# PABannier/bark.cpp

Measured on NVIDIA H100. Metric: audio sec/sec (inverse RTF), bark-small f16, batch 1 per GPU, semantic->coarse->fine->encodec, higher is better.
Workload: dtype f16 weights/operands, f32 accumulate (reference arithmetic)

## Files before the change

bark.cpp_b200/csrc/decode_kernels.cu:

```cuda
#include "epilogue.cuh"
#include "gpt_kernels.h"

namespace bark {

namespace {

constexpr int kThreads = 512;
constexpr int kWarps = kThreads / 32;
static_assert(kWarps == 16, "the soft_max tile is 16 columns wide: one warp finishes one column");
constexpr int kWarpSlotBytes = 12 * 1024;
constexpr int kHalfSlotBytes = kWarpSlotBytes / 2;
constexpr int kReplicas = kDecodeReplicas;

struct SmemLayout {
    static constexpr int wslot = 0;
    static constexpr int act = wslot + kWarps * kWarpSlotBytes;
    static constexpr int x = act + 4096 * 4;
    static constexpr int q = x + 1024 * 4;
    static constexpr int part = q + 1024 * 4;
    static constexpr int red = part + (32 * 16 + 128) * 4;
    static constexpr int sched = red + (kWarps + kWarps / 2 + kWarps + 4) * 8;
    static constexpr int total = sched + 128 * 32;
};

__device__ __forceinline__ uint32_t smem_u32(const void * p) { return (uint32_t) __cvta_generic_to_shared(p); }
__device__ __forceinline__ void mbar_init(uint32_t bar, uint32_t count) { asm volatile("mbarrier.init.shared::cta.b64 [%0], %1;" ::"r"(bar), "r"(count)); }
__device__ __forceinline__ void mbar_arrive(uint32_t bar) { asm volatile("mbarrier.arrive.shared::cta.b64 _, [%0];" ::"r"(bar) : "memory"); }
__device__ __forceinline__ void mbar_expect_tx(uint32_t bar, uint32_t bytes) { asm volatile("mbarrier.arrive.expect_tx.shared::cta.b64 _, [%0], %1;" ::"r"(bar), "r"(bytes) : "memory"); }
__device__ __forceinline__ void mbar_wait(uint32_t bar, uint32_t parity) {
    uint32_t done;
    asm volatile("{\n\t.reg .pred p;\n\tmbarrier.try_wait.parity.shared::cta.b64 p, [%1], %2;\n\tselp.u32 %0, 1, 0, p;\n\t}" : "=r"(done) : "r"(bar), "r"(parity) : "memory");
    if (done) return;
    const long long t0 = clock64();
    while (!done) {
        asm volatile("{\n\t.reg .pred p;\n\tmbarrier.try_wait.parity.shared::cta.b64 p, [%1], %2;\n\tselp.u32 %0, 1, 0, p;\n\t}" : "=r"(done) : "r"(bar), "r"(parity) : "memory");
        if (!done && clock64() - t0 > 4000000000ll) __trap();
    }
}
__device__ __forceinline__ void tma_bulk_g2s_stream(uint32_t dst, const void * src, uint32_t bytes, uint32_t bar, unsigned long long policy) {
    asm volatile("cp.async.bulk.shared::cluster.global.mbarrier::complete_tx::bytes.L2::cache_hint [%0], [%1], %2, [%3], %4;"
                 ::"r"(dst), "l"(src), "r"(bytes), "r"(bar), "l"(policy) : "memory");
}
__device__ __forceinline__ unsigned long long l2_evict_first_policy() {
    unsigned long long pol; asm volatile("createpolicy.fractional.L2::evict_first.b64 %0, 1.0;" : "=l"(pol));
    return pol;
}

typedef unsigned long long tagged_t;
__device__ __forceinline__ void publish(tagged_t * p, float v, uint32_t tag) {
    const tagged_t w = ((tagged_t) tag << 32) | (tagged_t) __float_as_uint(v);
    asm volatile("st.relaxed.gpu.global.u64 [%0], %1;" ::"l"(p), "l"(w) : "memory");
}
__device__ __forceinline__ tagged_t peek(const tagged_t * p) {
    tagged_t w;
    asm volatile("ld.relaxed.gpu.global.u64 %0, [%1];" : "=l"(w) : "l"(p) : "memory");
    return w;
}
__device__ __forceinline__ void peek2(const tagged_t * p, tagged_t & a, tagged_t & b) {
    asm volatile("ld.relaxed.gpu.global.v2.u64 {%0, %1}, [%2];" : "=l"(a), "=l"(b) : "l"(p) : "memory");
}
__device__ __forceinline__ void publish_all(tagged_t * base, int n, int i, float v, uint32_t tag, int lane) {
    if (lane < kReplicas) publish(base + (size_t) lane * n + i, v, tag);
}
__shared__ unsigned s_poll_ns;
enum { XT_Q = 0, XT_ATT = 1, XT_X1 = 2, XT_FF = 3, XT_X2 = 4, XT_SC = 5, XT_COUNT = 6 };
__shared__ unsigned s_headstart[XT_COUNT];
__device__ __forceinline__ float consume1(const tagged_t * p, uint32_t tag) {
    tagged_t w = peek(p);
    while ((uint32_t)(w >> 32) != tag) { __nanosleep(s_poll_ns); w = peek(p); }
    return __uint_as_float((uint32_t) w);
}
__device__ __forceinline__ int act_index(int k) {
    const int v = k & 31, c = k >> 5, g = c >> 3, e = c & 7;
    return (((g << 1) + (e >> 2)) * 32 + v) * 4 + (e & 3);
}

__shared__ unsigned long long * s_tim;
__shared__ int s_tim_layer, s_tim_tid;
template <bool TM>
__device__ __forceinline__ void tstamp(int i) {
    if (TM && s_tim && (int) threadIdx.x == s_tim_tid) {
        unsigned long long t; asm volatile("mov.u64 %0, %%globaltimer;" : "=l"(t));
        const int layer = s_tim_layer;
        if (blockIdx.x == 0) s_tim[layer * 32 + i] = t;
        if (layer == 5) s_tim[(64 + blockIdx.x) * 32 + i] = t;
    }
}

template <bool TM>
__device__ __forceinline__ void tstamp2(int row0, int i) {
    if (TM && s_tim && (int) threadIdx.x == s_tim_tid && blockIdx.x == 0 && s_tim_layer < 16) {
        unsigned long long t; asm volatile("mov.u64 %0, %%globaltimer;" : "=l"(t));
        s_tim[(row0 + s_tim_layer) * 32 + i] = t;
    }
}

enum { SINK_PLAIN = 0, SINK_ACT = 1, SINK_ACT_R16 = 2 };
template <int MAXJ>
__device__ __forceinline__ void consume_to_smem_inl(const tagged_t * g, int n, uint32_t tag, float * dst, int mode, int xt) {
    constexpr int PJ = MAXJ / 2;
    tagged_t w[PJ][2];
    g += (size_t)(blockIdx.x % kReplicas) * n;
    const unsigned hs = s_headstart[xt];
    if (hs) __nanosleep(hs);
#pragma unroll
    for (int j = 0; j < PJ; j++) { const int i = 2 * (threadIdx.x + j * kThreads); if (i < n) peek2(g + i, w[j][0], w[j][1]); }
#pragma unroll
    for (int j = 0; j < PJ; j++) {
        const int i = 2 * (threadIdx.x + j * kThreads);
        if (i < n) {
            while ((uint32_t)(w[j][0] >> 32) != tag || (uint32_t)(w[j][1] >> 32) != tag) { __nanosleep(s_poll_ns); peek2(g + i, w[j][0], w[j][1]); }
#pragma unroll
            for (int e = 0; e < 2; e++) {
                const float v = __uint_as_float((uint32_t) w[j][e]);
                if (mode == SINK_PLAIN) dst[i + e] = v; else dst[act_index(i + e)] = mode == SINK_ACT_R16 ? round_f16(v) : v;
            }
        }
    }
    __syncthreads();
}
__device__ __forceinline__ void consume_row_to_smem(const tagged_t * g, int n, uint32_t tag, float * dst) {
    tagged_t w[2];
    const unsigned hs = s_headstart[XT_SC];
    if (hs) __nanosleep(hs);
#pragma unroll
    for (int j = 0; j < 2; j++) { const int i = threadIdx.x + j * kThreads; if (i < n) w[j] = peek(g + i); }
#pragma unroll
    for (int j = 0; j < 2; j++) {
        const int i = threadIdx.x + j * kThreads;
        if (i < n) {
            while ((uint32_t)(w[j] >> 32) != tag) { __nanosleep(s_poll_ns); w[j] = peek(g + i); }
            dst[i] = __uint_as_float((uint32_t) w[j]);
        }
    }
    __syncthreads();
}
template <int MAXJ>
__device__ __noinline__ void consume_to_smem(const tagged_t * g, int n, uint32_t tag, float * dst, int mode, int xt) {
    consume_to_smem_inl<MAXJ>(g, n, tag, dst, mode, xt);
}


__device__ __forceinline__ double approx_rcp(double x) {
    double y = (double) __frcp_rn((float) x);
    double e = __fma_rn(-x, y, 1.0); y = __fma_rn(y, e, y);
    e = __fma_rn(-x, y, 1.0);        y = __fma_rn(y, e, y);
    return y;
}

template <bool ROUND16, bool TM, bool NATURAL = false, int COPY = 0>
__device__ __noinline__ void block_layernorm(const float * xs, int E, double inv_E, const float * __restrict__ g, const float * __restrict__ b, float * act,
                                             double * red, unsigned * fallback_counter, int sb) {
    const int tid = threadIdx.x, lane = tid & 31, warp = tid >> 5;
    const int tb = sb == 1 ? 0 : 16;
    tstamp2<TM>(48, tb + 0);
    double * sA = red, * sB = red + kWarps + kWarps / 2;
    float * fA = reinterpret_cast<float *>(red + kWarps);
    const int i0 = tid, i1 = tid + kThreads;
    const bool h0 = i0 < E, h1 = i1 < E;
    const float g0 = h0 ? __ldg(g + i0) : 0.f, g1 = h1 ? __ldg(g + i1) : 0.f;
    const float b0 = (b && h0) ? __ldg(b + i0) : 0.f, b1 = (b && h1) ? __ldg(b + i1) : 0.f;
    const float x0 = h0 ? xs[i0] : 0.f, x1 = h1 ? xs[i1] : 0.f;
    const double slack = 2.0 * (double) E * 0x1p-53 * (1.0 + 1e-6);

    double s = (double) x0 + (double) x1;
    float a = fabsf(x0) + fabsf(x1);
#pragma unroll
    for (int o = 16; o > 0; o >>= 1) { s += __shfl_xor_sync(0xffffffffu, s, o); a += __shfl_xor_sync(0xffffffffu, a, o); }
    tstamp2<TM>(48, tb + 1);
    if (lane == 0) { sA[warp] = s; fA[warp] = a; }
    __syncthreads();
    tstamp2<TM>(48, tb + 2);
    float mean;
    {
        double qd[1]; float qf[1];
        qd[0] = sA[lane & (kWarps - 1)]; qf[0] = fA[lane & (kWarps - 1)];
#pragma unroll
        for (int o = kWarps / 2; o > 0; o >>= 1) { qd[0] += __shfl_xor_sync(0xffffffffu, qd[0], o); qf[0] += __shfl_xor_sync(0xffffffffu, qf[0], o); }
        const double S = qd[0]; const float A = qf[0];
        if (S == 1.25) tstamp2<TM>(48, tb + 15);
        tstamp2<TM>(48, tb + 3);
        const double c = S * inv_E;
        const double hw = (slack * (double) A * 1.001) * inv_E + fabs(c) * 0x1p-50;
        mean = __double2float_rn(c - hw);
        if (mean != __double2float_rn(c + hw)) {
            double ss = 0.0;
            for (int i = 0; i < E; i++) ss = __dadd_rn(ss, (double) xs[i]);
            mean = __double2float_rn(__ddiv_rn(ss, (double) E));
            if (fallback_counter && tid == 0) atomicAdd(fallback_counter, 1u);
        }
    }
    tstamp<TM>(sb);
    const float v0 = __fsub_rn(x0, mean), v1 = __fsub_rn(x1, mean);
    double s2 = (h0 ? (double) __fmul_rn(v0, v0) : 0.0) + (h1 ? (double) __fmul_rn(v1, v1) : 0.0);
#pragma unroll
    for (int o = 16; o > 0; o >>= 1) s2 += __shfl_xor_sync(0xffffffffu, s2, o);
    if (s2 == 1.25) tstamp2<TM>(48, tb + 15);
    tstamp2<TM>(48, tb + 5);
    if (lane == 0) sB[warp] = s2;
    __syncthreads();
    tstamp2<TM>(48, tb + 6);
    float scale;
    {
        double qd[1];
        qd[0] = sB[lane & (kWarps - 1)];
#pragma unroll
        for (int o = kWarps / 2; o > 0; o >>= 1) qd[0] += __shfl_xor_sync(0xffffffffu, qd[0], o);
        const double S2 = qd[0];
        const double c = S2 * inv_E;
        const double hw = (slack * S2) * inv_E + c * 0x1p-50;
        float variance = __double2float_rn(c - hw);
        if (variance != __double2float_rn(c + hw)) {
            double ss = 0.0;
            for (int i = 0; i < E; i++) { const float v = __fsub_rn(xs[i], mean); ss = __dadd_rn(ss, (double) __fmul_rn(v, v)); }
            variance = __double2float_rn(__ddiv_rn(ss, (double) E));
            if (fallback_counter && tid == 0) atomicAdd(fallback_counter, 1u);
        }
        scale = __fdiv_rn(1.0f, __fsqrt_rn(__fadd_rn(variance, 1e-5f)));
    }
    if (scale == 1.25f) tstamp2<TM>(48, tb + 15);
    tstamp2<TM>(48, tb + 7);
    if (h0) { float y = __fmul_rn(__fmul_rn(v0, scale), g0); if (b) y = __fadd_rn(y, b0); act[NATURAL ? i0 : act_index(i0)] = ROUND16 ? round_f16(y) : y; }
    if (h1) { float y = __fmul_rn(__fmul_rn(v1, scale), g1); if (b) y = __fadd_rn(y, b1); act[NATURAL ? i1 : act_index(i1)] = ROUND16 ? round_f16(y) : y; }
    tstamp2<TM>(48, tb + 8);
    __syncthreads();
    tstamp2<TM>(48, tb + 9);
}

struct PhaseSched { int r0, r1, K, row_bytes; const unsigned char * w; const unsigned char * ws; };

enum { EP_QKV = 0, EP_RESID = 1, EP_GELU = 2, EP_LOGITS = 3 };

__device__ __forceinline__ float gelu_sel(float v, __half t) { return v <= -10.0f ? 0.0f : v >= 10.0f ? v : __half2float(t); }

template <typename WT> struct Unpack;
template <> struct Unpack<__half> {
    static constexpr int G = 8;
    __device__ static void w(const uint4 & u, float (&f)[8]) {
        const __half2 * h = reinterpret_cast<const __half2 *>(&u);
#pragma unroll
        for (int i = 0; i < 4; i++) { const float2 t = __half22float2(h[i]); f[2 * i] = t.x; f[2 * i + 1] = t.y; }
    }
};
template <> struct Unpack<float> {
    static constexpr int G = 4;
    __device__ static void w(const uint4 & u, float (&f)[4]) { f[0] = __uint_as_float(u.x); f[1] = __uint_as_float(u.y); f[2] = __uint_as_float(u.z); f[3] = __uint_as_float(u.w); }
};

__device__ __forceinline__ uint4 lds128(uint32_t addr) {
    uint4 v; asm volatile("ld.shared.v4.u32 {%0, %1, %2, %3}, [%4];" : "=r"(v.x), "=r"(v.y), "=r"(v.z), "=r"(v.w) : "r"(addr));
    return v;
}
template <typename WT, bool SH, int NR>
__device__ __forceinline__ void row_dot(const unsigned char * row, int row_bytes, const float * act, int K, int lane, float (&out)[NR]) {
    constexpr int G = Unpack<WT>::G;
    const int nsteps = K >> 5;
    const uint4 * wv = reinterpret_cast<const uint4 *>(row) + lane;
    const uint32_t sw = SH ? smem_u32(row) + lane * 16 : 0u;
    const int rstride = row_bytes >> 4;
    auto fetch = [&](int n, int i) -> uint4 { return SH ? lds128(sw + n * row_bytes + i * 512) : wv[n * rstride + i * 32]; };
    float acc[NR];
#pragma unroll
    for (int n = 0; n < NR; n++) acc[n] = 0.0f;
    if constexpr (G == 8) {
        const int ng = nsteps >> 3, tail = nsteps & 7;
#pragma unroll 3
        for (int g = 0; g < ng; g++) {
            const float4 a0 = *reinterpret_cast<const float4 *>(act + ((g * 2) * 32 + lane) * 4);
            const float4 a1 = *reinterpret_cast<const float4 *>(act + ((g * 2 + 1) * 32 + lane) * 4);
#pragma unroll
            for (int n = 0; n < NR; n++) {
                float w[8]; Unpack<WT>::w(fetch(n, g), w);
                float c = acc[n];
                c = __fmaf_rn(w[0], a0.x, c); c = __fmaf_rn(w[1], a0.y, c); c = __fmaf_rn(w[2], a0.z, c); c = __fmaf_rn(w[3], a0.w, c);
                c = __fmaf_rn(w[4], a1.x, c); c = __fmaf_rn(w[5], a1.y, c); c = __fmaf_rn(w[6], a1.z, c); c = __fmaf_rn(w[7], a1.w, c);
                acc[n] = c;
            }
        }
        if (tail) {
            const float * a0 = act + ((ng * 2) * 32 + lane) * 4, * a1 = act + ((ng * 2 + 1) * 32 + lane) * 4;
#pragma unroll
            for (int n = 0; n < NR; n++) {
                float w[8]; Unpack<WT>::w(fetch(n, ng), w);
#pragma unroll
                for (int e = 0; e < 8; e++) if (e < tail) acc[n] = __fmaf_rn(w[e], e < 4 ? a0[e] : a1[e - 4], acc[n]);
            }
        }
    } else {
        const int nq = nsteps >> 2, tail = nsteps & 3;
        for (int qd = 0; qd < nq; qd++) {
            const float4 a = *reinterpret_cast<const float4 *>(act + (qd * 32 + lane) * 4);
#pragma unroll
            for (int n = 0; n < NR; n++) {
                float w[4]; Unpack<WT>::w(fetch(n, qd), w);
                float c = acc[n];
                c = __fmaf_rn(w[0], a.x, c); c = __fmaf_rn(w[1], a.y, c); c = __fmaf_rn(w[2], a.z, c); c = __fmaf_rn(w[3], a.w, c);
                acc[n] = c;
            }
        }
        if (tail) {
            const float * a = act + (nq * 32 + lane) * 4;
#pragma unroll
            for (int n = 0; n < NR; n++) {
                float w[4]; Unpack<WT>::w(fetch(n, nq), w);
#pragma unroll
                for (int e = 0; e < 4; e++) if (e < tail) acc[n] = __fmaf_rn(w[e], a[e], acc[n]);
            }
        }
    }
#pragma unroll
    for (int n = 0; n < NR; n++) out[n] = lane_tree_reduce(acc[n]);
}

struct Q4 {};
template <typename WT> struct IsQ4 { static constexpr bool v = false; };
template <> struct IsQ4<Q4> { static constexpr bool v = true; };

__device__ __forceinline__ void quantize_act_q8(const float * act, int K, int8_t * q, float * d) {
    const int lane = threadIdx.x & 31, warp = threadIdx.x >> 5;
    for (int b = warp; b < (K >> 5); b += kWarps) {
        const float v = act[b * 32 + lane];
        float amax = fabsf(v);
#pragma unroll
        for (int o = 16; o > 0; o >>= 1) amax = fmaxf(amax, __shfl_xor_sync(0xffffffffu, amax, o));
        const float id = amax != 0.0f ? __fdiv_rn(127.0f, amax) : 0.0f;
        const float p = __fmul_rn(v, id);
        q[b * 32 + lane] = (int8_t)(isfinite(p) ? __float2int_rn(p) : -128);
        if (lane == 0) d[b] = __half2float(__float2half_rn(__fdiv_rn(amax, 127.0f)));
    }
    __syncthreads();
}

template <bool SH>
__device__ __forceinline__ float row_dot_q4(const unsigned char * qrows, const unsigned char * srows, int nrows, int nb, const int8_t * aq, const float * ad, int lane) {
    const int l = lane & 7, row = min(lane >> 3, nrows - 1);
    const bool high = l >= 4;
    const unsigned char * wq = qrows + (size_t) row * nb * 16 + (l & 3) * 4;
    const unsigned char * ws = srows + (size_t) row * nb * 2;
    const uint32_t s_wq = SH ? smem_u32(wq) : 0u, s_ws = SH ? smem_u32(ws) : 0u, s_aq = smem_u32(aq) + l * 4, s_ad = smem_u32(ad);
    float acc = 0.0f;
    constexpr int UB = 8;
    for (int b0 = 0; b0 < nb; b0 += UB) {
        uint32_t wr[UB]; float dr[UB]; int yr[UB];
#pragma unroll
        for (int u = 0; u < UB; u++) if (b0 + u < nb) {
            unsigned short hs; float da;
            if (SH) { asm volatile("ld.shared.u32 %0, [%1];" : "=r"(wr[u]) : "r"(s_wq + (b0 + u) * 16) : "memory"); asm volatile("ld.shared.u16 %0, [%1];" : "=h"(hs) : "r"(s_ws + (b0 + u) * 2) : "memory"); }
            else    { wr[u] = __ldg(reinterpret_cast<const uint32_t *>(wq + (size_t)(b0 + u) * 16)); hs = __ldg(reinterpret_cast<const unsigned short *>(ws + (size_t)(b0 + u) * 2)); }
            asm volatile("ld.shared.f32 %0, [%1];" : "=f"(da) : "r"(s_ad + (b0 + u) * 4) : "memory");
            asm volatile("ld.shared.s32 %0, [%1];" : "=r"(yr[u]) : "r"(s_aq + (b0 + u) * 32) : "memory");
            dr[u] = __fmul_rn(__half2float(__ushort_as_half(hs)), da);
        }
#pragma unroll
        for (int u = 0; u < UB; u++) {
            if (b0 + u < nb) {
                const uint32_t w = (high ? (wr[u] >> 4) : wr[u]) & 0x0f0f0f0fu;
                const int wi = (int) __vsub4(w, 0x08080808u);
                acc = __fmaf_rn(dr[u], (float) __dp4a(wi, yr[u], 0), acc);
            }
        }
    }
    acc = __fadd_rn(acc, __shfl_xor_sync(0xffffffffu, acc, 4));
    acc = __fadd_rn(acc, __shfl_xor_sync(0xffffffffu, acc, 2));
    acc = __fadd_rn(acc, __shfl_xor_sync(0xffffffffu, acc, 1));
    return acc;
}
__device__ __forceinline__ float wte_q4_value(const void * wte, int E, int row, int i) {
    const unsigned char * blk = (const unsigned char *) wte + ((size_t) row * (E >> 5) + (i >> 5)) * 18;
    const float d = __half2float(__ushort_as_half((unsigned short)(blk[0] | (blk[1] << 8))));
    const int j = i & 31, q = j < 16 ? (blk[2 + j] & 0x0f) : (blk[2 + j - 16] >> 4);
    return __fmul_rn((float)(q - 8), d);
}

template <typename WT>
__device__ __forceinline__ void embed_token(const void * wte, const float * wpe, const int32_t * token_ptr, int token, int n_vocab_in, int E, int n_past, float * xs) {
    if (token_ptr) token = min(max(__ldcg(token_ptr), 0), n_vocab_in - 1);
    for (int i = threadIdx.x; i < E; i += kThreads) {
        float t;
        if constexpr (IsQ4<WT>::v) t = wte_q4_value(wte, E, token, i);
        else t = (float) ((const WT *) wte)[(size_t) token * E + i];
        xs[i] = __fadd_rn(t, wpe[(size_t) n_past * E + i]);
    }
}

constexpr int kMaxTasks = 8;

struct BlockCtx {
    tagged_t * gq, * gk, * gv, * gx, * gff, * gatt, * gscores;
    float * mem_k, * mem_v, * logits;
    const __half * gelu_tab;
    unsigned long long policy;
    int E, ctx, n_past, n_phases;
    float scale;
};
__shared__ BlockCtx s_bc;
__shared__ __align__(8) unsigned long long s_bar[kWarps][2];
extern __shared__ __align__(128) unsigned char dsm[];

__device__ __forceinline__ const PhaseSched * sched_tab() { return reinterpret_cast<const PhaseSched *>(dsm + SmemLayout::sched); }
__device__ __forceinline__ void warp_rows(const PhaseSched & p, int warp, int & a, int & b) {
    const int n = p.r1 - p.r0;
    a = p.r0 + ((warp * n) >> 4); b = p.r0 + (((warp + 1) * n) >> 4);
}

__device__ __forceinline__ bool q4_staged(uint32_t qbytes, uint32_t sbytes, const unsigned char * ssrc) {
    return qbytes != 0 && qbytes + sbytes <= (uint32_t) kHalfSlotBytes && (sbytes & 15u) == 0 && (reinterpret_cast<uintptr_t>(ssrc) & 15u) == 0;
}

__device__ __forceinline__ void stage_rows(int phase) {
    if (phase >= s_bc.n_phases || (threadIdx.x & 31) != 0) return;
    const int warp = threadIdx.x >> 5, half = phase & 1;
    const PhaseSched p = sched_tab()[phase];
    int a, b; warp_rows(p, warp, a, b);
    const uint32_t bytes = (uint32_t)((b - a) * p.row_bytes);
    const uint32_t bar = smem_u32(&s_bar[warp][half]);
    const uint32_t dst = smem_u32(dsm + SmemLayout::wslot) + warp * kWarpSlotBytes + half * kHalfSlotBytes;
    if (p.ws) {
        const uint32_t sbytes = (uint32_t)((b - a) * (p.K >> 5) * 2);
        const unsigned char * ssrc = p.ws + (size_t) a * (p.K >> 5) * 2;
        if (q4_staged(bytes, sbytes, ssrc)) {
            asm volatile("fence.proxy.async.shared::cta;" ::: "memory");
            mbar_expect_tx(bar, bytes + sbytes);
            tma_bulk_g2s_stream(dst, p.w + (size_t) a * p.row_bytes, bytes, bar, s_bc.policy);
            tma_bulk_g2s_stream(dst + bytes, ssrc, sbytes, bar, s_bc.policy);
        } else {
            mbar_arrive(bar);
        }
        return;
    }
    if (bytes != 0 && bytes <= (uint32_t) kHalfSlotBytes) {
        asm volatile("fence.proxy.async.shared::cta;" ::: "memory");
        mbar_expect_tx(bar, bytes);
        tma_bulk_g2s_stream(dst, p.w + (size_t) a * p.row_bytes, bytes, bar, s_bc.policy);
    } else {
        mbar_arrive(bar);
    }
}

__device__ __forceinline__ uint32_t staged_bytes_of(int phase, int warp) {
    const PhaseSched p = sched_tab()[phase];
    int a, b; warp_rows(p, warp, a, b);
    const uint32_t bytes = (uint32_t)((b - a) * p.row_bytes);
    if (p.ws) {
        const uint32_t sbytes = (uint32_t)((b - a) * (p.K >> 5) * 2);
        return q4_staged(bytes, sbytes, p.ws + (size_t) a * (p.K >> 5) * 2) ? bytes + sbytes : 0u;
    }
    return bytes <= (uint32_t) kHalfSlotBytes ? bytes : 0u;
}
__device__ __forceinline__ void cp_async_16(uint32_t dst, const float * src) { asm volatile("cp.async.cg.shared.global [%0], [%1], 16;" ::"r"(dst), "l"(src) : "memory"); }
__device__ __forceinline__ void cp_async_commit() { asm volatile("cp.async.commit_group;" ::: "memory"); }
__device__ __forceinline__ void cp_async_wait_all() { asm volatile("cp.async.wait_group 0;" ::: "memory"); }

template <typename WT, bool TM>
__device__ __noinline__ void run_phase(int phase, int ep, int layer, uint32_t otag, int sb) {
    const int lane = threadIdx.x & 31, warp = threadIdx.x >> 5;
    const int tb = sb == 3 ? 0 : sb == 18 ? 8 : sb == 24 ? 16 : 24;
    tstamp2<TM>(32, tb + 0);
    const PhaseSched p = sched_tab()[phase];
    const float * act = reinterpret_cast<const float *>(dsm + SmemLayout::act);
    const float * xs = reinterpret_cast<const float *>(dsm + SmemLayout::x);
    const int half = phase & 1;
    int a, b; warp_rows(p, warp, a, b);
    const uint32_t bytes = (uint32_t)((b - a) * p.row_bytes);
    const bool staged = bytes != 0 && bytes <= (uint32_t) kHalfSlotBytes;
    const unsigned char * slot = dsm + SmemLayout::wslot + (size_t) warp * kWarpSlotBytes + (size_t) half * kHalfSlotBytes;
    mbar_wait(smem_u32(&s_bar[warp][half]), (uint32_t)(phase >> 1) & 1u);
    tstamp<TM>(sb);
    const int E = s_bc.E;
    auto emit = [&](int r, float v) {
        if (ep == EP_QKV) {
            const size_t slot_off = ((size_t) layer * s_bc.ctx + s_bc.n_past) * E;
            if (r < E) publish_all(s_bc.gq, E, r, v, otag, lane);
            else if (lane == 0) {
                if (r < 2 * E) { publish(s_bc.gk + (r - E), v, otag); s_bc.mem_k[slot_off + (r - E)] = v; }
                else           { publish(s_bc.gv + (r - 2 * E), v, otag); s_bc.mem_v[slot_off + (r - 2 * E)] = v; }
            }
        } else if (ep == EP_RESID) {
            publish_all(s_bc.gx, E, r, __fadd_rn(v, xs[r]), otag, lane);
        } else if (lane == 0) {
            s_bc.logits[r] = v;
        }
    };
    if constexpr (IsQ4<WT>::v) {
        const int nb = p.K >> 5;
        const int8_t * aq = reinterpret_cast<const int8_t *>(dsm + SmemLayout::q);
        const float * ad = reinterpret_cast<const float *>(dsm + SmemLayout::part) + 512;
        const uint32_t sbytes = (uint32_t)((b - a) * nb * 2);
        const unsigned char * ssrc = p.ws + (size_t) a * nb * 2;
        const bool st4 = q4_staged(bytes, sbytes, ssrc);
        for (int r = a; r < b; r += 4) {
            const int n = min(4, b - r);
            const float t = st4 ? row_dot_q4<true>(slot + (size_t)(r - a) * p.row_bytes, slot + bytes + (size_t)(r - a) * nb * 2, n, nb, aq, ad, lane)
                                : row_dot_q4<false>(p.w + (size_t) r * p.row_bytes, p.ws + (size_t) r * nb * 2, n, nb, aq, ad, lane);
#pragma unroll
            for (int g = 0; g < 4; g++) {
                const float v = __shfl_sync(0xffffffffu, t, g * 8);
                if (g < n && lane < kReplicas) {
                    if (ep == EP_GELU) publish_all(s_bc.gff, 4 * E, r + g, gelu_sel(v, s_bc.gelu_tab[__half_as_ushort(__float2half_rn(v))]), otag, lane);
                    else emit(r + g, v);
                }
            }
        }
        __syncwarp();
        tstamp<TM>(sb + 1);
        return;
    } else {
    int j = 0;
    tstamp2<TM>(32, tb + 1);
    for (int r = a; r < b;) {
        const unsigned char * row = staged ? slot + (size_t) j * p.row_bytes : p.w + (size_t) r * p.row_bytes;
        if (r + 1 < b) {
            float v[2];
            if (staged) row_dot<WT, true, 2>(row, p.row_bytes, act, p.K, lane, v);
            else { float u[1]; row_dot<WT, false, 1>(row, p.row_bytes, act, p.K, lane, u); v[0] = u[0]; row_dot<WT, false, 1>(row + p.row_bytes, p.row_bytes, act, p.K, lane, u); v[1] = u[0]; }
            if (v[0] == 1.2345e30f) tstamp2<TM>(32, tb + 7);
            tstamp2<TM>(32, tb + 2);
            if (lane < kReplicas) {
                if (ep == EP_GELU) {
                    const __half t0 = s_bc.gelu_tab[__half_as_ushort(__float2half_rn(v[0]))], t1 = s_bc.gelu_tab[__half_as_ushort(__float2half_rn(v[1]))];
                    publish_all(s_bc.gff, 4 * E, r, gelu_sel(v[0], t0), otag, lane); publish_all(s_bc.gff, 4 * E, r + 1, gelu_sel(v[1], t1), otag, lane);
                } else { emit(r, v[0]); emit(r + 1, v[1]); }
            }
            tstamp2<TM>(32, tb + 3);
            r += 2; j += 2;
        } else {
            float v[1];
            if (staged) row_dot<WT, true, 1>(row, p.row_bytes, act, p.K, lane, v); else row_dot<WT, false, 1>(row, p.row_bytes, act, p.K, lane, v);
            if (v[0] == 1.2345e30f) tstamp2<TM>(32, tb + 7);
            tstamp2<TM>(32, tb + 4);
            if (lane < kReplicas) {
                if (ep == EP_GELU) publish_all(s_bc.gff, 4 * E, r, gelu_sel(v[0], s_bc.gelu_tab[__half_as_ushort(__float2half_rn(v[0]))]), otag, lane);
                else emit(r, v[0]);
            }
            tstamp2<TM>(32, tb + 5);
            r += 1; j += 1;
        }
    }
    __syncwarp();
    tstamp<TM>(sb + 1);
    }
}

}

template <int DSTEPS>
__device__ __forceinline__ void key_tail(int warp, uint32_t & off, int & cap) {
    constexpr int D = DSTEPS * 32;
    off = (max(staged_bytes_of(0, warp), staged_bytes_of(2, warp)) + 127u) & ~127u;
    cap = min(2 * kMaxTasks, (int)(((uint32_t) kHalfSlotBytes - min(off, (uint32_t) kHalfSlotBytes)) / (uint32_t)(D * 4)));
}

template <int DSTEPS>
__device__ __noinline__ void p2_stage_keys(int layer, int H, int n_kv, unsigned score_cta0) {
    constexpr int D = DSTEPS * 32, GPT = D / 4;
    const int lane = threadIdx.x & 31, warp = threadIdx.x >> 5;
    const int E = s_bc.E, ctx = s_bc.ctx, n_past = s_bc.n_past;
    uint32_t off; int cap; key_tail<DSTEPS>(warp, off, cap);
    const float * Kc = s_bc.mem_k + (size_t) layer * ctx * E;
    const int total = H * n_past, gw = (int)(blockIdx.x - score_cta0) * kWarps + warp, nw = (int)(gridDim.x - score_cta0) * kWarps;
    const uint32_t dst = smem_u32(dsm + SmemLayout::wslot + (size_t) warp * kWarpSlotBytes + off);
#pragma unroll 2
    for (int q = lane; q < cap * GPT; q += 32) {
        const int i = q / GPT, g = q - i * GPT, t = gw + i * nw;
        if (t < total) {
            const int h = t / n_past, k = t - h * n_past;
            cp_async_16(dst + (uint32_t) q * 16u, Kc + (size_t) k * E + h * D + g * 4);
        }
    }
    cp_async_commit();
}

template <int DSTEPS, bool TM>
__device__ __noinline__ void p2_scores(int il, int H, int n_kv, uint32_t t_qkv, uint32_t t_sc, unsigned score_cta0) {
    constexpr int D = DSTEPS * 32;
    const int lane = threadIdx.x & 31, warp = threadIdx.x >> 5;
    const int E = s_bc.E, ctx = s_bc.ctx, n_past = s_bc.n_past;
    const float scale = s_bc.scale;
    float * qs = reinterpret_cast<float *>(dsm + SmemLayout::q);
    const float * Kc = s_bc.mem_k + (size_t) il * ctx * E;
    const int total = H * n_past, gw = (int)(blockIdx.x - score_cta0) * kWarps + warp, nw = (int)(gridDim.x - score_cta0) * kWarps;
    const int sq = nw / n_past, sr = nw - sq * n_past;
    uint32_t off; int cap; key_tail<DSTEPS>(warp, off, cap);
    if (score_cta0 == 0) cap = 0;
    const float * ks = reinterpret_cast<const float *>(dsm + SmemLayout::wslot + (size_t) warp * kWarpSlotBytes + off) + lane;
    tstamp<TM>(6);
    consume_to_smem<2>(s_bc.gq, E, t_qkv, qs, SINK_PLAIN, XT_Q);
    tstamp<TM>(7);
    if (cap > 0) { cp_async_wait_all(); __syncwarp(); }
    int h = gw / n_past, k = gw - h * n_past;
    int done = 0;
#pragma unroll 1
    for (int b0 = 0; b0 < cap && gw + b0 * nw < total; b0 += kMaxTasks) {
        float r[kMaxTasks];
#pragma unroll
        for (int i = 0; i < kMaxTasks; i++) {
            float acc = 0.0f;
            if (b0 + i < cap && h < H) {
#pragma unroll
                for (int c = 0; c < DSTEPS; c++) acc = __fmaf_rn(ks[(b0 + i) * D + c * 32], qs[h * D + c * 32 + lane], acc);
            }
            r[i] = acc;
            k += sr; h += sq; if (k >= n_past) { k -= n_past; h++; }
        }
        static_assert(kMaxTasks == 8, "the transposed butterfly below is written for eight tasks");
        const bool u16 = (lane & 16) != 0, u8 = (lane & 8) != 0, u4 = (lane & 4) != 0;
#pragma unroll
        for (int i = 0; i < 4; i++) { const float keep = u16 ? r[i + 4] : r[i], send = u16 ? r[i] : r[i + 4]; r[i] = __fadd_rn(keep, __shfl_xor_sync(0xffffffffu, send, 16)); }
#pragma unroll
        for (int i = 0; i < 2; i++) { const float keep = u8 ? r[i + 2] : r[i], send = u8 ? r[i] : r[i + 2]; r[i] = __fadd_rn(keep, __shfl_xor_sync(0xffffffffu, send, 8)); }
        { const float keep = u4 ? r[1] : r[0], send = u4 ? r[0] : r[1]; r[0] = __fadd_rn(keep, __shfl_xor_sync(0xffffffffu, send, 4)); }
        r[0] = __fadd_rn(r[0], __shfl_xor_sync(0xffffffffu, r[0], 1));
        r[0] = __fadd_rn(r[0], __shfl_xor_sync(0xffffffffu, r[0], 2));
        const int mine = b0 + (u16 ? 4 : 0) + (u8 ? 2 : 0) + (u4 ? 1 : 0);
        const int t = gw + mine * nw;
        if ((lane & 3) == 0 && mine < cap && t < total) {
            const int hh = t / n_past, kk = t - hh * n_past;
            publish(s_bc.gscores + (size_t) hh * ctx + kk, __fmul_rn(r[0], scale), t_sc);
        }
        done = min(b0 + kMaxTasks, cap);
    }
#pragma unroll 1
    for (int t = gw + done * nw; t < total; t += nw) {
        const int hh = t / n_past, kk = t - hh * n_past;
        float acc = 0.0f;
#pragma unroll
        for (int c = 0; c < DSTEPS; c++) acc = __fmaf_rn(__ldcg(Kc + (size_t) kk * E + hh * D + c * 32 + lane), qs[hh * D + c * 32 + lane], acc);
        const float rr = lane_tree_reduce(acc);
        if (lane == 0) publish(s_bc.gscores + (size_t) hh * ctx + kk, __fmul_rn(rr, scale), t_sc);
    }
#pragma unroll 1
    for (int hh = gw; hh < H; hh += nw) {
        float acc = 0.0f;
#pragma unroll
        for (int c = 0; c < DSTEPS; c++) acc = __fmaf_rn(consume1(s_bc.gk + hh * D + c * 32 + lane, t_qkv), qs[hh * D + c * 32 + lane], acc);
        const float rr = lane_tree_reduce(acc);
        if (lane == 0) publish(s_bc.gscores + (size_t) hh * ctx + n_past, __fmul_rn(rr, scale), t_sc);
    }
}

template <bool TM>
__device__ __forceinline__ float softmax_exp_rcp(float * p, int n_kv, double * red, unsigned * fallbacks) {
    const int tid = threadIdx.x, lane = tid & 31, warp = tid >> 5;
    float * bc = reinterpret_cast<float *>(red + kWarps + kWarps / 2 + kWarps);
    float mx = __int_as_float(0xff800000);
#pragma unroll 1
    for (int i = tid; i < n_kv; i += kThreads) mx = fmaxf(mx, p[i]);
#pragma unroll
    for (int o = 16; o > 0; o >>= 1) mx = fmaxf(mx, __shfl_xor_sync(0xffffffffu, mx, o));
    float * fred = reinterpret_cast<float *>(red);
    if (lane == 0) fred[warp] = mx;
    __syncthreads();
    mx = fred[0];
#pragma unroll
    for (int w = 1; w < kWarps; w++) mx = fmaxf(mx, fred[w]);
    tstamp<TM>(11);
    const int nchunks = n_kv >> 3, n8 = nchunks << 3;
#pragma unroll 1
    for (int i = tid; i < n_kv; i += kThreads) {
        const float d = __fsub_rn(p[i], mx);
        p[i] = i < n8 ? ggml_v_expf_dev(d) : glibc_expf_dev(d);
    }
    __syncthreads();
    tstamp<TM>(12);
    if (warp == 0) {
        auto chunk_sum = [&](int c) {
            const float4 lo4 = *reinterpret_cast<const float4 *>(p + c * 8), hi4 = *reinterpret_cast<const float4 *>(p + c * 8 + 4);
            const float t0 = __fadd_rn(hi4.x, lo4.x), t1 = __fadd_rn(hi4.y, lo4.y), t2 = __fadd_rn(hi4.z, lo4.z), t3 = __fadd_rn(hi4.w, lo4.w);
            return __fadd_rn(__fadd_rn(t0, t2), __fadd_rn(t1, t3));
        };
        double s = 0.0;
#pragma unroll 1
        for (int c = lane; c < nchunks; c += 32) s += (double) chunk_sum(c);
#pragma unroll
        for (int o = 16; o > 0; o >>= 1) s += __shfl_xor_sync(0xffffffffu, s, o);
        if (lane == 0) {
            const double dl = 2.0 * (double)(nchunks + 8) * 0x1p-53 * s * (1.0 + 1e-6);
            double lo = s - dl, hi = s + dl;
#pragma unroll 1
            for (int i = n8; i < n_kv; i++) { const double tl = (double) p[i]; lo = __dadd_rn(lo, tl); hi = __dadd_rn(hi, tl); }
            const double mid = 0.5 * (lo + hi), y = approx_rcp(mid);
            const double rw = (hi - lo) * y * 0.5 + 0x1p-48;
            float f_lo = __double2float_rn(y * (1.0 - rw));
            const float f_hi = __double2float_rn(y * (1.0 + rw));
            if (f_lo != f_hi) {
                double q2 = 0.0;
#pragma unroll 1
                for (int c = 0; c < nchunks; c++) q2 = __dadd_rn(q2, (double) chunk_sum(c));
#pragma unroll 1
                for (int i = n8; i < n_kv; i++) q2 = __dadd_rn(q2, (double) p[i]);
                f_lo = __double2float_rn(__ddiv_rn(1.0, q2));
                if (fallbacks) atomicAdd(fallbacks + 1, 1u);
            }
            bc[2] = f_lo;
        }
    }
    __syncthreads();
    tstamp<TM>(13);
    return bc[2];
}

template <int DSTEPS, bool TM>
__device__ __noinline__ void p3_attention(int il, int n_kv, uint32_t t_qkv, uint32_t t_sc, uint32_t t_att, unsigned * ln_fallbacks) {
    constexpr int D = DSTEPS * 32;
    const int tid = threadIdx.x, lane = tid & 31, warp = tid >> 5;
    const int E = s_bc.E, ctx = s_bc.ctx, n_past = s_bc.n_past;
    float * act = reinterpret_cast<float *>(dsm + SmemLayout::act);
    float * qs = reinterpret_cast<float *>(dsm + SmemLayout::q);
    float * part = reinterpret_cast<float *>(dsm + SmemLayout::part);
    double * red = reinterpret_cast<double *>(dsm + SmemLayout::red);
    struct { float * mem_v; unsigned * ln_fallbacks; } A{s_bc.mem_v, ln_fallbacks};
    constexpr int parts = D >> 4;
    const int pv_h = blockIdx.x / parts, pv_c = blockIdx.x % parts, np = n_kv & ~31;
    const int v = tid >> 4, dd = tid & 15, h = pv_h;
    const int col0 = pv_h * D + pv_c * 16;
    const int nstep = np >> 5, r = n_kv - np;
    const int nstep_all = nstep + (r > 0 ? 1 : 0);
    const float * Vt = A.mem_v + (size_t) il * ctx * E + col0;
    const uint32_t voff = (staged_bytes_of(4 * il + 1, warp) + 127u) & ~127u;
    const bool vs_ok = voff + (uint32_t) nstep_all * 128u <= (uint32_t) kHalfSlotBytes;
    const float * vs = reinterpret_cast<const float *>(dsm + SmemLayout::wslot + (size_t) warp * kWarpSlotBytes + kHalfSlotBytes + voff);
    if (vs_ok) {
        const uint32_t dst = smem_u32(vs);
        const int sub = lane >> 3, vl2 = (lane >> 2) & 1, g = lane & 3;
#pragma unroll 2
        for (int c0 = 0; c0 < nstep_all; c0 += 4) {
            const int c = c0 + sub, k = 2 * warp + vl2 + 32 * c;
            if (c < nstep_all && k < n_past) cp_async_16(dst + (uint32_t)(((c * 2 + vl2) * 16 + g * 4) * 4), Vt + (size_t) k * E + g * 4);
        }
        cp_async_commit();
    }
    const float v_new = consume1(s_bc.gv + col0 + dd, t_qkv);
    __syncthreads();
    tstamp<TM>(9);
    float * p = qs;
    consume_row_to_smem(s_bc.gscores + (size_t) h * ctx, n_kv, t_sc, p);
    tstamp<TM>(10);
    const float sc_f = softmax_exp_rcp<TM>(p, n_kv, red, A.ln_fallbacks);
    float acc = 0.0f;
    if (vs_ok) {
        cp_async_wait_all(); __syncwarp();
#pragma unroll 8
        for (int c = 0; c < nstep; c++) {
            const int k = v + 32 * c;
            const float vv = k < n_past ? vs[c * 32 + lane] : v_new;
            acc = __fmaf_rn(vv, __fmul_rn(p[k], sc_f), acc);
        }
    } else {
#pragma unroll 8
        for (int c = 0; c < nstep; c++) {
            const int k = v + 32 * c;
            const float vv = k < n_past ? __ldcg(Vt + (size_t) k * E + dd) : v_new;
            acc = __fmaf_rn(vv, __fmul_rn(p[k], sc_f), acc);
        }
    }
    part[v * 17 + dd] = acc;
    const int r8 = r & ~7, n4 = r8 + ((r - r8) >= 4 ? 4 : 0);
    if (v < r) {
        const float vv = (np + v < n_past) ? (vs_ok ? vs[nstep * 32 + lane] : __ldcg(Vt + (size_t)(np + v) * E + dd)) : v_new;
        act[v * 16 + dd] = v < n4 ? __fmul_rn(vv, __fmul_rn(p[np + v], sc_f)) : vv;
    }
    __syncthreads();
    tstamp<TM>(15);
    {
        float sum = lane_tree_reduce(part[lane * 17 + warp]);
#pragma unroll 8
        for (int j = 0; j < n4; j++) sum = __fadd_rn(sum, act[j * 16 + warp]);
#pragma unroll 1
        for (int j = n4; j < r; j++) sum = __fmaf_rn(act[j * 16 + warp], __fmul_rn(p[np + j], sc_f), sum);
        publish_all(s_bc.gatt, E, col0 + warp, sum, t_att, lane);
    }
    __syncthreads();
}

template <typename WT, int DSTEPS, bool TM>
__global__ void __launch_bounds__(kThreads, 1) gpt_decode_step_kernel(DecodeArgs A) {
    float * act = reinterpret_cast<float *>(dsm + SmemLayout::act);
    float * xs = reinterpret_cast<float *>(dsm + SmemLayout::x);
    float * qs = reinterpret_cast<float *>(dsm + SmemLayout::q);
    float * part = reinterpret_cast<float *>(dsm + SmemLayout::part);
    double * red = reinterpret_cast<double *>(dsm + SmemLayout::red);
    float * bc = reinterpret_cast<float *>(red + kWarps + kWarps / 2 + kWarps);
    const int tid = threadIdx.x, lane = tid & 31, warp = tid >> 5;
    constexpr int D = DSTEPS * 32;
    const int E = A.E, H = A.H, L = A.L, ctx = A.block_size, n_past = A.n_past, n_kv = n_past + 1;
    constexpr bool kQ4 = IsQ4<WT>::v;
    constexpr bool kRound = !kQ4 && sizeof(WT) == 2;
    constexpr int kSinkAct = kQ4 ? SINK_PLAIN : kRound ? SINK_ACT_R16 : SINK_ACT;
    int8_t * act_q = reinterpret_cast<int8_t *>(dsm + SmemLayout::q);
    float * act_d = reinterpret_cast<float *>(dsm + SmemLayout::part) + 512;

    PhaseSched * sched = reinterpret_cast<PhaseSched *>(dsm + SmemLayout::sched);
    const int n_phases = 4 * L + 1;
    if (tid < n_phases) {
        const DecodePhase ph = A.phases[tid];
        int lo = 0, hi = ph.n_out;
        if (tid == n_phases - 1) { lo = A.lm_lo; hi = A.lm_hi; }
        const int n = hi - lo, G = gridDim.x, base = n / G, rem = n % G, cta = blockIdx.x;
        PhaseSched e;
        e.r0 = lo + cta * base + min(cta, rem); e.r1 = e.r0 + base + (cta < rem ? 1 : 0);
        e.K = ph.K; e.row_bytes = ph.row_bytes; e.w = (const unsigned char *) ph.w; e.ws = (const unsigned char *) ph.ws;
        sched[tid] = e;
    }
    if (tid == kThreads - 1) {
        s_bc.gq = (tagged_t *) A.gq; s_bc.gk = (tagged_t *) A.gk; s_bc.gv = (tagged_t *) A.gv; s_bc.gx = (tagged_t *) A.gx; s_bc.gff = (tagged_t *) A.gff;
        s_bc.gatt = (tagged_t *) A.gatt; s_bc.gscores = (tagged_t *) A.gscores;
        s_bc.mem_k = A.mem_k; s_bc.mem_v = A.mem_v; s_bc.logits = A.logits; s_bc.gelu_tab = A.gelu_tab;
        s_bc.policy = l2_evict_first_policy();
        s_bc.E = E; s_bc.ctx = ctx; s_bc.n_past = n_past; s_bc.n_phases = n_phases; s_bc.scale = 1.0f / sqrtf((float) E / (float) H);
        s_tim = A.timing; s_tim_layer = 0; s_tim_tid = A.timing_tid; s_poll_ns = A.poll_ns;
    }
    if (tid < XT_COUNT) {
        const bool pv = (int) blockIdx.x < A.H * ((A.E / A.H) >> 4);
        s_headstart[tid] = (tid == XT_ATT && pv) ? 0u : A.headstart[tid];
    }
    if (lane == 0) {
        mbar_init(smem_u32(&s_bar[warp][0]), 1); mbar_init(smem_u32(&s_bar[warp][1]), 1);
        asm volatile("fence.mbarrier_init.release.cluster;" ::: "memory");
    }
    __syncthreads();
    stage_rows(0);
    stage_rows(1);

    embed_token<WT>(A.wte, A.wpe, A.token_ptr, A.token, A.n_vocab_in, E, n_past, xs);
    __syncthreads();

    uint32_t tag = A.tag_base;
    const double inv_E = A.inv_E;

    const int parts = D >> 4;
    const bool pv_cta = (int) blockIdx.x < H * parts;
    const unsigned score_cta0 = (gridDim.x >= (unsigned)(H * parts + 64)) ? (unsigned)(H * parts) : 0u;
    const bool score_cta = blockIdx.x >= score_cta0;

    if (score_cta0 != 0 && score_cta) p2_stage_keys<DSTEPS>(0, H, n_kv, score_cta0);
#pragma unroll 1
    for (int il = 0; il < L; il++) {
        const DecodeLayerVec lv = A.layer_vecs[il];
        const uint32_t t_qkv = tag + 1, t_sc = tag + 2, t_att = tag + 3, t_x1 = tag + 4, t_ff = tag + 5, t_x2 = tag + 6;
        tag += 6;
        if (tid == A.timing_tid) s_tim_layer = il;
        tstamp<TM>(0);
        block_layernorm<kRound, TM, kQ4>(xs, E, inv_E, lv.ln_1_g, lv.ln_1_b, act, red, A.ln_fallbacks, 1);
        if constexpr (kQ4) quantize_act_q8(act, E, act_q, act_d);
        tstamp<TM>(2);
        run_phase<WT, TM>(4 * il + 0, EP_QKV, il, t_qkv, 3);

        if constexpr (kQ4) __syncthreads();
        if (score_cta) {
            p2_scores<DSTEPS, TM>(il, H, n_kv, t_qkv, t_sc, score_cta0);
            tstamp<TM>(8);
            if (score_cta0 != 0 && il + 1 < L) p2_stage_keys<DSTEPS>(il + 1, H, n_kv, score_cta0);
        } else {
            tstamp<TM>(8);
        }
        if (pv_cta) p3_attention<DSTEPS, TM>(il, n_kv, t_qkv, t_sc, t_att, A.ln_fallbacks);
        tstamp<TM>(16);
        stage_rows(4 * il + 2);

        consume_to_smem<2>(s_bc.gatt, E, t_att, act, kSinkAct, XT_ATT);
        if constexpr (kQ4) quantize_act_q8(act, E, act_q, act_d);
        tstamp<TM>(17);
        run_phase<WT, TM>(4 * il + 1, EP_RESID, il, t_x1, 18);

        consume_to_smem<2>(s_bc.gx, E, t_x1, xs, SINK_PLAIN, XT_X1);
        stage_rows(4 * il + 3);
        tstamp<TM>(21);
        block_layernorm<kRound, TM, kQ4>(xs, E, inv_E, lv.ln_2_g, lv.ln_2_b, act, red, A.ln_fallbacks, 22);
        if constexpr (kQ4) quantize_act_q8(act, E, act_q, act_d);
        tstamp<TM>(23);
        run_phase<WT, TM>(4 * il + 2, EP_GELU, il, t_ff, 24);
        __syncthreads();
        tstamp<TM>(27);

        consume_to_smem<8>(s_bc.gff, 4 * E, t_ff, act, kSinkAct, XT_FF);
        stage_rows(4 * il + 4);
        if constexpr (kQ4) quantize_act_q8(act, 4 * E, act_q, act_d);
        tstamp<TM>(28);
        run_phase<WT, TM>(4 * il + 3, EP_RESID, il, t_x2, 29);

        consume_to_smem<2>(s_bc.gx, E, t_x2, xs, SINK_PLAIN, XT_X2);
        stage_rows(4 * il + 5);
        tstamp<TM>(14);
    }
    if (tid == A.timing_tid) s_tim_layer = L;
    tstamp<TM>(0);
    block_layernorm<kRound, TM, kQ4>(xs, E, inv_E, A.ln_f_g, A.ln_f_b, act, red, A.ln_fallbacks, 1);
    if constexpr (kQ4) quantize_act_q8(act, E, act_q, act_d);
    tstamp<TM>(2);
    run_phase<WT, TM>(4 * L, EP_LOGITS, 0, 0, 3);
}

__global__ void __launch_bounds__(kThreads) decode_rows_kernel(int op, const float * __restrict__ x, int n, double inv_n, const float * __restrict__ g,
                                                               const float * __restrict__ b, float * __restrict__ out, unsigned * counters) {
    __shared__ double red[kWarps + kWarps / 2 + kWarps + 4];
    __shared__ __align__(16) float p[1024];
    const float * xr = x + (size_t) blockIdx.x * n;
    float * orow = out + (size_t) blockIdx.x * n;
    if (op == 0) { block_layernorm<false, false, true, 1>(xr, n, inv_n, g, b, orow, red, counters, 1); return; }
    for (int i = threadIdx.x; i < n; i += kThreads) p[i] = xr[i];
    __syncthreads();
    const float sc_f = softmax_exp_rcp<false>(p, n, red, counters);
    for (int i = threadIdx.x; i < n; i += kThreads) orow[i] = __fmul_rn(p[i], sc_f);
}

void decode_rows(int op, const float * x, int rows, int n, const float * g, const float * b, float * out, unsigned * counters, cudaStream_t s) {
    BARK_LAUNCH(decode_rows_kernel, rows, kThreads, 0, s, op, x, n, 1.0 / n, g, b, out, counters);
}

template <bool SH>
__global__ void __launch_bounds__(kThreads) decode_q4_rows_kernel(const float * __restrict__ x, int K, const unsigned char * __restrict__ wq,
                                                                  const unsigned char * __restrict__ ws, int n_out, MatmulEpilogue ep,
                                                                  int8_t * __restrict__ q_out, float * __restrict__ d_out) {
    const int lane = threadIdx.x & 31, warp = threadIdx.x >> 5, nb = K >> 5;
    int8_t * aq = reinterpret_cast<int8_t *>(dsm);
    float * ad = reinterpret_cast<float *>(dsm + K);
    unsigned char * slot = dsm + K + nb * 4 + (size_t) warp * 4 * nb * 18;
    quantize_act_q8(x, K, aq, ad);
    for (int i = threadIdx.x; i < K; i += kThreads) q_out[i] = aq[i];
    for (int i = threadIdx.x; i < nb; i += kThreads) d_out[i] = ad[i];
    for (int r = warp * 4; r < n_out; r += kWarps * 4) {
        const int n = min(4, n_out - r);
        float t;
        if constexpr (SH) {
            const uint32_t * src = reinterpret_cast<const uint32_t *>(wq + (size_t) r * nb * 16);
            const unsigned short * ssrc = reinterpret_cast<const unsigned short *>(ws + (size_t) r * nb * 2);
            for (int i = lane; i < n * nb * 4; i += 32) reinterpret_cast<uint32_t *>(slot)[i] = src[i];
            for (int i = lane; i < n * nb; i += 32) reinterpret_cast<unsigned short *>(slot + n * nb * 16)[i] = ssrc[i];
            __syncwarp();
            t = row_dot_q4<true>(slot, slot + n * nb * 16, n, nb, aq, ad, lane);
            __syncwarp();
        } else {
            t = row_dot_q4<false>(wq + (size_t) r * nb * 16, ws + (size_t) r * nb * 2, n, nb, aq, ad, lane);
        }
#pragma unroll
        for (int g = 0; g < 4; g++) {
            const float v = __shfl_sync(0xffffffffu, t, g * 8);
            if (lane == 0 && g < n) matmul_epilogue(ep, 0, r + g, v);
        }
    }
}

void decode_q4_rows(bool staged, const float * x, int K, const void * qs, const void * scales, int n_out, const MatmulEpilogue & ep, int8_t * q_out,
                    float * d_out, cudaStream_t s) {
    const size_t smem = (size_t) K + (K >> 5) * 4 + (staged ? (size_t) kWarps * 4 * (K >> 5) * 18 : 0);
    const unsigned char * wq = (const unsigned char *) qs, * ws = (const unsigned char *) scales;
    if (staged) {
        BARK_CUDA_CHECK(cudaFuncSetAttribute(decode_q4_rows_kernel<true>, cudaFuncAttributeMaxDynamicSharedMemorySize, (int) smem));
        BARK_LAUNCH(decode_q4_rows_kernel<true>, 1, kThreads, smem, s, x, K, wq, ws, n_out, ep, q_out, d_out);
    } else {
        BARK_LAUNCH(decode_q4_rows_kernel<false>, 1, kThreads, smem, s, x, K, wq, ws, n_out, ep, q_out, d_out);
    }
}

static size_t decode_smem_bytes() { return (size_t) SmemLayout::total + 128; }

int decode_tags_per_step(int n_layer) { return 6 * n_layer; }

template <typename WT, int DSTEPS, bool TM>
static void launch_variant(DecodeArgs a, int n_sm, cudaStream_t s) {
    static std::atomic<unsigned long long> configured{0};
    if (first_use_on_this_device(configured))
        BARK_CUDA_CHECK(cudaFuncSetAttribute(gpt_decode_step_kernel<WT, DSTEPS, TM>, cudaFuncAttributeMaxDynamicSharedMemorySize, (int) decode_smem_bytes()));
    void * kargs[] = {(void *) &a};
    BARK_CUDA_CHECK(cudaLaunchCooperativeKernel((const void *) gpt_decode_step_kernel<WT, DSTEPS, TM>, dim3(n_sm), dim3(kThreads), kargs, decode_smem_bytes(), s));
}
template <typename WT, int DSTEPS>
static void launch_one(DecodeArgs a, int n_sm, cudaStream_t s) {
    if (a.timing) launch_variant<WT, DSTEPS, true>(a, n_sm, s); else launch_variant<WT, DSTEPS, false>(a, n_sm, s);
}

void launch_decode_step(const DecodeArgs & args, WType wt, int n_sm, cudaStream_t s) {
    const int dsteps = args.E / args.H / 32;
    if (g_prof_on) prof_begin("gpt_decode_step_kernel", s, g_next_bytes, g_next_flops);
    if (wt == W_Q4_0) {
        switch (dsteps) { case 1: launch_one<Q4, 1>(args, n_sm, s); break; case 2: launch_one<Q4, 2>(args, n_sm, s); break;
                          case 3: launch_one<Q4, 3>(args, n_sm, s); break; default: launch_one<Q4, 4>(args, n_sm, s); }
    } else if (wt == W_F16) {
        switch (dsteps) { case 1: launch_one<__half, 1>(args, n_sm, s); break; case 2: launch_one<__half, 2>(args, n_sm, s); break;
                          case 3: launch_one<__half, 3>(args, n_sm, s); break; default: launch_one<__half, 4>(args, n_sm, s); }
    } else {
        switch (dsteps) { case 1: launch_one<float, 1>(args, n_sm, s); break; case 2: launch_one<float, 2>(args, n_sm, s); break;
                          case 3: launch_one<float, 3>(args, n_sm, s); break; default: launch_one<float, 4>(args, n_sm, s); }
    }
    if (g_prof_on) prof_end(s);
    g_next_bytes = g_next_flops = 0.0;
    ++g_kernel_launches;
}

}
```

Before: 13.24.

## Pack attention and GELU outputs as half pairs in tagged exchange words

In the rounded f16 path, the attention and FFN-GELU outputs are now published as two f16 values per 64-bit tagged word instead of one f32 per word. This halves the cross-CTA exchange traffic and polling, which are likely latency-bound. The GELU phase row partition is aligned to pairs (gsh) so each warp emits whole pairs, and attention staging goes through shared memory with an extra __syncthreads. It relies on the f16 rounding already applied by the consumer, so results should match, but the extra sync and the packing work add some overhead.

New measurement: 13.41 (median of 6 runs). 1.01x the previous value.

```diff
diff --git a/bark.cpp_b200/csrc/decode_kernels.cu b/bark.cpp_b200/csrc/decode_kernels.cu
--- a/bark.cpp_b200/csrc/decode_kernels.cu
+++ b/bark.cpp_b200/csrc/decode_kernels.cu
@@ -11,6 +11,8 @@
 constexpr int kWarpSlotBytes = 12 * 1024;
 constexpr int kHalfSlotBytes = kWarpSlotBytes / 2;
 constexpr int kReplicas = kDecodeReplicas;
+
+struct PhaseSched { int r0, r1, K, row_bytes, gsh; const unsigned char * w; const unsigned char * ws; };
 
 struct SmemLayout {
     static constexpr int wslot = 0;
@@ -20,7 +22,7 @@
     static constexpr int part = q + 1024 * 4;
     static constexpr int red = part + (32 * 16 + 128) * 4;
     static constexpr int sched = red + (kWarps + kWarps / 2 + kWarps + 4) * 8;
-    static constexpr int total = sched + 128 * 32;
+    static constexpr int total = sched + 128 * (int) sizeof(PhaseSched);
 };
 
 __device__ __forceinline__ uint32_t smem_u32(const void * p) { return (uint32_t) __cvta_generic_to_shared(p); }
@@ -47,10 +49,11 @@
 }
 
 typedef unsigned long long tagged_t;
-__device__ __forceinline__ void publish(tagged_t * p, float v, uint32_t tag) {
-    const tagged_t w = ((tagged_t) tag << 32) | (tagged_t) __float_as_uint(v);
+__device__ __forceinline__ void publish_word(tagged_t * p, uint32_t payload, uint32_t tag) {
+    const tagged_t w = ((tagged_t) tag << 32) | (tagged_t) payload;
     asm volatile("st.relaxed.gpu.global.u64 [%0], %1;" ::"l"(p), "l"(w) : "memory");
 }
+__device__ __forceinline__ void publish(tagged_t * p, float v, uint32_t tag) { publish_word(p, __float_as_uint(v), tag); }
 __device__ __forceinline__ tagged_t peek(const tagged_t * p) {
     tagged_t w;
     asm volatile("ld.relaxed.gpu.global.u64 %0, [%1];" : "=l"(w) : "l"(p) : "memory");
@@ -61,6 +64,10 @@
 }
 __device__ __forceinline__ void publish_all(tagged_t * base, int n, int i, float v, uint32_t tag, int lane) {
     if (lane < kReplicas) publish(base + (size_t) lane * n + i, v, tag);
+}
+__device__ __forceinline__ void publish_all_pair(tagged_t * base, int n, int i, float v0, float v1, uint32_t tag, int lane) {
+    const uint32_t h = (uint32_t) __half_as_ushort(__float2half_rn(v0)) | ((uint32_t) __half_as_ushort(__float2half_rn(v1)) << 16);
+    if (lane < kReplicas) publish_word(base + (size_t) lane * n + i, h, tag);
 }
 __shared__ unsigned s_poll_ns;
 enum { XT_Q = 0, XT_ATT = 1, XT_X1 = 2, XT_FF = 3, XT_X2 = 4, XT_SC = 5, XT_COUNT = 6 };
@@ -114,6 +121,29 @@
             for (int e = 0; e < 2; e++) {
                 const float v = __uint_as_float((uint32_t) w[j][e]);
                 if (mode == SINK_PLAIN) dst[i + e] = v; else dst[act_index(i + e)] = mode == SINK_ACT_R16 ? round_f16(v) : v;
+            }
+        }
+    }
+    __syncthreads();
+}
+__device__ __noinline__ void consume_pairs_to_smem(const tagged_t * g, int nw, uint32_t tag, float * dst, int xt) {
+    constexpr int PJ = 2;
+    tagged_t w[PJ][2];
+    g += (size_t)(blockIdx.x % kReplicas) * nw;
+    const unsigned hs = s_headstart[xt];
+    if (hs) __nanosleep(hs);
+#pragma unroll
+    for (int j = 0; j < PJ; j++) { const int i = 2 * (threadIdx.x + j * kThreads); if (i < nw) peek2(g + i, w[j][0], w[j][1]); }
+#pragma unroll
+    for (int j = 0; j < PJ; j++) {
+        const int i = 2 * (threadIdx.x + j * kThreads);
+        if (i < nw) {
+            while ((uint32_t)(w[j][0] >> 32) != tag || (uint32_t)(w[j][1] >> 32) != tag) { __nanosleep(s_poll_ns); peek2(g + i, w[j][0], w[j][1]); }
+#pragma unroll
+            for (int e = 0; e < 2; e++) {
+                const uint32_t h = (uint32_t) w[j][e];
+                dst[act_index(2 * (i + e))] = __half2float(__ushort_as_half((unsigned short)(h & 0xffffu)));
+                dst[act_index(2 * (i + e) + 1)] = __half2float(__ushort_as_half((unsigned short)(h >> 16)));
             }
         }
     }
@@ -227,8 +257,6 @@
     tstamp2<TM>(48, tb + 9);
 }
 
-struct PhaseSched { int r0, r1, K, row_bytes; const unsigned char * w; const unsigned char * ws; };
-
 enum { EP_QKV = 0, EP_RESID = 1, EP_GELU = 2, EP_LOGITS = 3 };
 
 __device__ __forceinline__ float gelu_sel(float v, __half t) { return v <= -10.0f ? 0.0f : v >= 10.0f ? v : __half2float(t); }
@@ -399,8 +427,8 @@
 
 __device__ __forceinline__ const PhaseSched * sched_tab() { return reinterpret_cast<const PhaseSched *>(dsm + SmemLayout::sched); }
 __device__ __forceinline__ void warp_rows(const PhaseSched & p, int warp, int & a, int & b) {
-    const int n = p.r1 - p.r0;
-    a = p.r0 + ((warp * n) >> 4); b = p.r0 + (((warp + 1) * n) >> 4);
+    const int n = (p.r1 - p.r0) >> p.gsh;
+    a = p.r0 + (((warp * n) >> 4) << p.gsh); b = p.r0 + ((((warp + 1) * n) >> 4) << p.gsh);
 }
 
 __device__ __forceinline__ bool q4_staged(uint32_t qbytes, uint32_t sbytes, const unsigned char * ssrc) {
@@ -455,6 +483,7 @@
 __device__ __noinline__ void run_phase(int phase, int ep, int layer, uint32_t otag, int sb) {
     const int lane = threadIdx.x & 31, warp = threadIdx.x >> 5;
     const int tb = sb == 3 ? 0 : sb == 18 ? 8 : sb == 24 ? 16 : 24;
+    constexpr bool kPacked = !IsQ4<WT>::v && sizeof(WT) == 2;
     tstamp2<TM>(32, tb + 0);
     const PhaseSched p = sched_tab()[phase];
     const float * act = reinterpret_cast<const float *>(dsm + SmemLayout::act);
@@ -518,7 +547,8 @@
             if (lane < kReplicas) {
                 if (ep == EP_GELU) {
                     const __half t0 = s_bc.gelu_tab[__half_as_ushort(__float2half_rn(v[0]))], t1 = s_bc.gelu_tab[__half_as_ushort(__float2half_rn(v[1]))];
-                    publish_all(s_bc.gff, 4 * E, r, gelu_sel(v[0], t0), otag, lane); publish_all(s_bc.gff, 4 * E, r + 1, gelu_sel(v[1], t1), otag, lane);
+                    if constexpr (kPacked) publish_all_pair(s_bc.gff, 2 * E, r >> 1, gelu_sel(v[0], t0), gelu_sel(v[1], t1), otag, lane);
+                    else { publish_all(s_bc.gff, 4 * E, r, gelu_sel(v[0], t0), otag, lane); publish_all(s_bc.gff, 4 * E, r + 1, gelu_sel(v[1], t1), otag, lane); }
                 } else { emit(r, v[0]); emit(r + 1, v[1]); }
             }
             tstamp2<TM>(32, tb + 3);
@@ -699,7 +729,7 @@
     return bc[2];
 }
 
-template <int DSTEPS, bool TM>
+template <int DSTEPS, bool TM, bool PACK>
 __device__ __noinline__ void p3_attention(int il, int n_kv, uint32_t t_qkv, uint32_t t_sc, uint32_t t_att, unsigned * ln_fallbacks) {
     constexpr int D = DSTEPS * 32;
     const int tid = threadIdx.x, lane = tid & 31, warp = tid >> 5;
@@ -767,6 +797,13 @@
         for (int j = 0; j < n4; j++) sum = __fadd_rn(sum, act[j * 16 + warp]);
 #pragma unroll 1
         for (int j = n4; j < r; j++) sum = __fmaf_rn(act[j * 16 + warp], __fmul_rn(p[np + j], sc_f), sum);
+        if constexpr (PACK) {
+            float * s_att = reinterpret_cast<float *>(red);
+            if (lane == 0) s_att[warp] = sum;
+            __syncthreads();
+            if (warp < kWarps / 2) publish_all_pair(s_bc.gatt, E / 2, (col0 >> 1) + warp, s_att[2 * warp], s_att[2 * warp + 1], t_att, lane);
+            return;
+        }
         publish_all(s_bc.gatt, E, col0 + warp, sum, t_att, lane);
     }
     __syncthreads();
@@ -795,10 +832,11 @@
         const DecodePhase ph = A.phases[tid];
         int lo = 0, hi = ph.n_out;
         if (tid == n_phases - 1) { lo = A.lm_lo; hi = A.lm_hi; }
-        const int n = hi - lo, G = gridDim.x, base = n / G, rem = n % G, cta = blockIdx.x;
+        const int gsh = (kRound && tid < n_phases - 1 && (tid & 3) == 2) ? 1 : 0;
+        const int n = (hi - lo) >> gsh, G = gridDim.x, base = n / G, rem = n % G, cta = blockIdx.x;
         PhaseSched e;
-        e.r0 = lo + cta * base + min(cta, rem); e.r1 = e.r0 + base + (cta < rem ? 1 : 0);
-        e.K = ph.K; e.row_bytes = ph.row_bytes; e.w = (const unsigned char *) ph.w; e.ws = (const unsigned char *) ph.ws;
+        e.r0 = lo + ((cta * base + min(cta, rem)) << gsh); e.r1 = e.r0 + ((base + (cta < rem ? 1 : 0)) << gsh);
+        e.gsh = gsh; e.K = ph.K; e.row_bytes = ph.row_bytes; e.w = (const unsigned char *) ph.w; e.ws = (const unsigned char *) ph.ws;
         sched[tid] = e;
     }
     if (tid == kThreads - 1) {
@@ -853,11 +891,12 @@
         } else {
             tstamp<TM>(8);
         }
-        if (pv_cta) p3_attention<DSTEPS, TM>(il, n_kv, t_qkv, t_sc, t_att, A.ln_fallbacks);
+        if (pv_cta) p3_attention<DSTEPS, TM, kRound>(il, n_kv, t_qkv, t_sc, t_att, A.ln_fallbacks);
         tstamp<TM>(16);
         stage_rows(4 * il + 2);
 
-        consume_to_smem<2>(s_bc.gatt, E, t_att, act, kSinkAct, XT_ATT);
+        if constexpr (kRound) consume_pairs_to_smem(s_bc.gatt, E / 2, t_att, act, XT_ATT);
+        else consume_to_smem<2>(s_bc.gatt, E, t_att, act, kSinkAct, XT_ATT);
         if constexpr (kQ4) quantize_act_q8(act, E, act_q, act_d);
         tstamp<TM>(17);
         run_phase<WT, TM>(4 * il + 1, EP_RESID, il, t_x1, 18);
@@ -872,7 +911,8 @@
         __syncthreads();
         tstamp<TM>(27);
 
-        consume_to_smem<8>(s_bc.gff, 4 * E, t_ff, act, kSinkAct, XT_FF);
+        if constexpr (kRound) consume_pairs_to_smem(s_bc.gff, 2 * E, t_ff, act, XT_FF);
+        else consume_to_smem<8>(s_bc.gff, 4 * E, t_ff, act, kSinkAct, XT_FF);
         stage_rows(4 * il + 4);
         if constexpr (kQ4) quantize_act_q8(act, 4 * E, act_q, act_d);
         tstamp<TM>(28);
```
